# imedslab/OAProgressionMMF

Measured on AMD Instinct MI355X. Metric: knees/sec full XR+MRI+clin fusion train step, higher is better.
Workload: dtype f32; 1 GPU; syn3: XR1MR3C1CnnTrf train step (fwd+FocalLoss+bwd+Adam), per-GPU batch 8, global batch 8, BASELINE config 4 on BASELINE's synthetic tensors: XR 1x310x310 + 3 x MRI 1x160x384x384 (slice-major) + 9 clinical; random-init weights; parallelism=dp1, activation_recompute=012,012,01

## Files before the change

oaprogressionmmf_amd/csrc/koaf_conv.hip:

```cpp
#include <string.h>
#include "koaf_common.h"
#include <stdlib.h>

namespace {

inline void zero_gemm(KoafGemm* g) { *g = KoafGemm{}; g->alpha = 1.f; g->nb0 = g->nb1 = 1; g->splitk = 1; }

inline int conv_out(int H, int K, int s, int p) { return (H + 2 * p - K) / s + 1; }

inline int64_t rup32(int64_t v) { return (v + 31) / 32 * 32; }

inline void set_fimg(KoafGemm* g, const KoafWImg* w, int R, int64_t K) {
    g->fmt = 1;
    g->A.fscale = KOAF_ACT_SCALE;
    g->B.amax = w->amax;
    if (!w->f) return;
    g->B.kind = 2; g->B.gather = 0;
    g->B.planes = w->f; g->B.ld = rup32(K); g->B.plane_stride = (int64_t)R * g->B.ld;
}

inline void set_aplanes(KoafOperand* a, const uint16_t* planes, int64_t plane_elems) {
    a->kind = 2; a->planes = planes; a->plane_stride = plane_elems; a->zeros = planes + 2 * plane_elems;
    a->ptr = nullptr; a->ptr2 = nullptr; a->tf = 0; a->sc = a->sh = a->sc2 = nullptr;
}
// ... 253 lines not shown
        g.A.ld = Cin;
    } else {
        g.A.gather = 1;
        g.A.H = H; g.A.W = W; g.A.C = Cin; g.A.CS = Cin;
        g.A.PH = OH; g.A.PW = OW;
        g.A.KH = KH; g.A.KW = KW; g.A.stride = stride; g.A.pad = pad; g.A.pad_w = pad;
    }
    if (in_sc) { g.A.tf = 1; g.A.sc = in_sc; g.A.sh = in_sh; }
    if (tail) { g.A.tf = 3; g.A.ptr2 = tail->idt; g.A.side = tail->y_out; g.A.sc2 = tail->idt_sc; g.A.sh2 = tail->idt_sc ? tail->idt_sh : nullptr; }
    g.B.ptr = w;
    g.B.kind = 0;
    g.B.ld = (int64_t)KH * KW * Cin;
    g.M = (int)M; g.N = Cout; g.K = KH * KW * Cin;
    if (wimg && wimg->amax) set_fimg(&g, wimg, Cout, g.K);
    if (x_planes) {
        KOAF_REQUIRE(g.A.gather == 1 && g.B.kind == 2, "koaf_conv2d_fwd: x_planes serve the gathered kernels and need wimg->f");
        set_aplanes(&g.A, x_planes, (int64_t)N * H * W * Cin);
    }
    g.C = y; g.ldc = Cout;
    g.stats = stats;
    g.stats_shift = stats ? stats_shift : nullptr;
    g.act16 = act16 ? 1 : 0;
    if (emit) {
        KOAF_REQUIRE(emit->planes && emit->sc && emit->sh && (Cout % 8) == 0, "koaf_conv2d_fwd: emit needs planes / sc / sh and Cout %% 8 == 0");
        g.out_planes = emit->planes; g.out_sc = emit->sc; g.out_sh = emit->sh; g.out_ps = M * Cout;
    }
    if (stats_rows) *stats_rows = koaf_gemm_part_rows(&g);
    return koaf_gemm(&g, stream);
}

extern "C" int32_t koaf_conv2d_stats_rows(int64_t M, int32_t Cout) { return (int32_t)cdiv64(M, 64); }

static void set_apply(KoafOperand* a, const KoafBnApply* ap, int C) {
    a->ptr = ap->dz; a->ptr2 = ap->c; a->tf = 2;
    a->sc = ap->coef; a->sc2 = ap->coef + 2 * (int64_t)C; a->sh = ap->coef + 3 * (int64_t)C;
    a->amax = ap->amax;
}

static void set_bnb(KoafGemm* g, const KoafBnb* b, float* part) {
    if (!b) return;
    g->bnb_amax = b->dz_amax;
    g->bnb_mode = b->mode;
    g->bnb_c = b->c; g->bnb_y = b->y; g->bnb_sc = b->sc; g->bnb_sh = b->sh;
    g->bnb_mean = b->mean; g->bnb_invstd = b->invstd;
    g->bnb2_c = b->c2; g->bnb2_mean = b->mean2; g->bnb2_invstd = b->invstd2;
    g->bnb_part = part;
}

extern "C" int32_t koaf_conv2d_dgrad_bnb_rows(int32_t N, int32_t H, int32_t W, int32_t Cin, int32_t stride) {
    if (stride == 2) {
        int64_t r = 0;
        for (int py = 0; py < 2; ++py)
            for (int px = 0; px < 2; ++px) r += cdiv64((int64_t)N * ((H - py + 1) / 2) * ((W - px + 1) / 2), 64);
        return (int32_t)r;
    }
    return (int32_t)cdiv64((int64_t)N * H * W, 64);
}

extern "C" int koaf_conv2d_dgrad_bnb(const float* dy, const float* w, float* dx, int32_t N, int32_t H, int32_t W,
                                     int32_t Cin, int32_t Cout, int32_t KH, int32_t KW, int32_t stride, int32_t pad,
                                     const float* residual, const KoafBnb* bnb, float* part, int32_t* part_rows,
                                     const KoafWImg* wimg, const float* dy_amax, const KoafBnApply* dy_apply,
                                     const uint16_t* dy_planes, int32_t act16, void* stream) {
    KOAF_REQUIRE(!dy_planes || (wimg && wimg->amax && wimg->d && (dy_amax || dy_apply) && KH * KW > 1),
                 "koaf_conv2d_dgrad: dy_planes need the weight's D plane image, dy_amax and a gathered (KH*KW > 1) kernel");
    KOAF_REQUIRE((dy || dy_apply || dy_planes) && w && dx && N > 0 && Cout % 32 == 0 && Cin % 4 == 0, "koaf_conv2d_dgrad: bad args");
    KOAF_REQUIRE(!dy_apply || (dy_apply->dz && dy_apply->c && dy_apply->coef && dy_apply->amax && wimg && wimg->amax && wimg->d),
                 "koaf_conv2d_dgrad: dy_apply needs dz / c / coef / amax and the weight's D plane image");
    if (dy_apply) { dy = dy_apply->dz; dy_amax = dy_apply->amax; }
    if (bnb && bnb->dz_amax && hipMemsetAsync(bnb->dz_amax, 0, sizeof(float), (hipStream_t)stream) != hipSuccess) {
        koaf_set_error("koaf_conv2d_dgrad_bnb: memset failed");
        return KOAF_ELAUNCH;
    }
    const bool f16 = wimg && wimg->amax && dy_amax;
    const bool ps = f16 && wimg->d != nullptr;
    const uint16_t* w_dimg = ps ? wimg->d : nullptr;
    const int64_t dld = (int64_t)KH * KW * Cout, dps = (int64_t)Cin * dld;
    KOAF_REQUIRE(!bnb || (part && part_rows), "koaf_conv2d_dgrad_bnb: part / part_rows required");
    const int nsum = (bnb && bnb->c2) ? 3 : 2;
    int rows_done = 0;
    const int OH = conv_out(H, KH, stride, pad), OW = conv_out(W, KW, stride, pad);
    const int64_t M = (int64_t)N * H * W;
    KOAF_REQUIRE(M < (1ll << 31), "koaf_conv2d_dgrad: too many pixels");
    KoafGemm g;
    if (stride == 2) {
        for (int py = 0; py < 2; ++py)
            for (int px = 0; px < 2; ++px) {
                const int Hc = (H - py + 1) / 2, Wc = (W - px + 1) / 2;
                if (Hc <= 0 || Wc <= 0) continue;
                const int khs = (py + pad) & 1, kws = (px + pad) & 1;
                const int nkh = khs < KH ? (KH - khs + 1) / 2 : 0, nkw = kws < KW ? (KW - kws + 1) / 2 : 0;
                const int offy = (py + pad - khs) / 2, offx = (px + pad - kws) / 2;
                zero_gemm(&g);
                g.prec = 1;
                if (f16) { g.fmt = 1; g.A.amax = dy_amax; g.B.amax = wimg->amax; }
                g.A.ptr = dy; g.A.kind = 0; g.A.gather = 2;
                if (dy_apply) set_apply(&g.A, dy_apply, Cout);
                g.A.H = OH; g.A.W = OW; g.A.C = Cout; g.A.CS = Cout;
                g.A.PH = Hc; g.A.PW = Wc;
                g.A.KH = nkh > 0 ? nkh : 1; g.A.KW = nkw > 0 ? nkw : 1; g.A.stride = 1; g.A.pad = offy; g.A.pad_w = offx;
                g.B.ptr = w + ((int64_t)khs * KW + kws) * Cin; g.B.kind = 1; g.B.gather = 3;
                g.B.C = Cout; g.B.ld = (int64_t)KH * KW * Cin;
                g.B.KW = g.A.KW; g.B.tap_stride = 2ll * Cin; g.B.tap_stride_h = 2ll * KW * Cin;
                if (ps) {
                    g.B.kind = 2; g.B.gather = 0;
                    g.B.planes = w_dimg + ((int64_t)khs * KW + kws) * Cout; g.B.ld = dld; g.B.plane_stride = dps;
                    g.B.tap_stride = 2ll * Cout; g.B.tap_stride_h = 2ll * KW * Cout;
                }
                if (dy_planes && nkh > 0 && nkw > 0) set_aplanes(&g.A, dy_planes, (int64_t)N * OH * OW * Cout);
                g.M = N * Hc * Wc; g.N = Cin; g.K = nkh * nkw * Cout;
                g.C = dx; g.ldc = Cin;
                g.residual = residual; g.ldr = Cin;
                g.cmap = 1; g.cm_PH = Hc; g.cm_PW = Wc; g.cm_H = H; g.cm_W = W; g.cm_py = py; g.cm_px = px;
                if (bnb) {
                    set_bnb(&g, bnb, part + (int64_t)rows_done * nsum * Cin);
                    rows_done += koaf_gemm_part_rows(&g);
                }
                g.act16 = act16 ? 2 : 0;
                int rc = koaf_gemm(&g, stream);
                if (rc != KOAF_OK) return rc;
            }
        if (part_rows) *part_rows = rows_done;
        return KOAF_OK;
    }
    zero_gemm(&g);
    g.prec = 1;
    if (f16) { g.fmt = 1; g.A.amax = dy_amax; g.B.amax = wimg->amax; }
    g.A.ptr = dy;
    g.A.kind = 0;
    if (dy_apply) set_apply(&g.A, dy_apply, Cout);
    g.B.ptr = w;
    g.B.kind = 1;
    if (KH == 1 && KW == 1 && stride == 1 && pad == 0) {
        g.A.gather = 0;
        g.A.ld = Cout;
        g.B.gather = 0;
        g.B.ld = Cin;
    } else {
        g.A.gather = 2;
        g.A.H = OH; g.A.W = OW; g.A.C = Cout; g.A.CS = Cout;
        g.A.PH = H; g.A.PW = W;
        g.A.KH = KH; g.A.KW = KW; g.A.stride = stride; g.A.pad = pad; g.A.pad_w = pad;
        g.B.gather = 3;
        g.B.C = Cout;
        g.B.ld = (int64_t)KH * KW * Cin;
        g.B.KW = KW;
        g.B.tap_stride = Cin;
        g.B.tap_stride_h = (int64_t)KW * Cin;
    }
    if (ps) {
        g.B.kind = 2; g.B.gather = 0; g.B.C = 0; g.B.tap_stride = g.B.tap_stride_h = 0;
        g.B.planes = w_dimg; g.B.ld = dld; g.B.plane_stride = dps;
    }
    if (dy_planes) set_aplanes(&g.A, dy_planes, (int64_t)N * OH * OW * Cout);
    g.M = (int)M; g.N = Cin; g.K = KH * KW * Cout;
    g.C = dx; g.ldc = Cin;
    g.residual = residual; g.ldr = Cin;
    if (bnb) {
        set_bnb(&g, bnb, part);
        *part_rows = koaf_gemm_part_rows(&g);
    }
    g.act16 = act16 ? 2 : 0;
    return koaf_gemm(&g, stream);
}

extern "C" int koaf_conv2d_dgrad(const float* dy, const float* w, float* dx, int32_t N, int32_t H, int32_t W,
                                 int32_t Cin, int32_t Cout, int32_t KH, int32_t KW, int32_t stride, int32_t pad,
                                 const float* residual, const KoafWImg* wimg, const float* dy_amax,
                                 const KoafBnApply* dy_apply, const uint16_t* dy_planes, int32_t act16, void* stream) {
    return koaf_conv2d_dgrad_bnb(dy, w, dx, N, H, W, Cin, Cout, KH, KW, stride, pad, residual, nullptr, nullptr,
                                 nullptr, wimg, dy_amax, dy_apply, dy_planes, act16, stream);
}

bool koaf_wgrad3_ring_ok(int N, int H, int W, int Cin, int Cout);
int64_t koaf_wgrad3_ring_ws(int N, int H, int W, int Cin, int Cout);
// ... 453 lines not shown
```

oaprogressionmmf_amd/models/_encoder.py:

```python
import os
from collections import namedtuple

import torch
from torch import nn

from .. import ops
from ..arena import deliver_grad, grad_target, packed_weight, weight_planes
from ._core_fes import BasicBlock, Bottleneck

USE_SIDE_STREAM = os.environ.get("KOAF_SIDE_STREAM", "1") != "0"


class _Rec:
    __slots__ = ("kind", "blk", "yin", "c1", "s1", "c2", "s2", "c3", "s3", "cd", "sd", "y", "dims", "wexp", "tail")

    def __init__(self):
        for k in self.__slots__:
            setattr(self, k, None)


def _stat_shift(bn, train):
    return bn.running_mean if (train and bn is not None and bn.running_mean is not None) else None


# ... 32 lines not shown
                                      tail_idsaved=tail.idsaved, emit=emit)
    elif g == 1:
        y, part = ops.conv2d_fwd(x, w, N, H, W, cin, cout, k, k, s, p, sc, sh, stats=train, shift=shift,
                                 wimg=weight_planes(conv.weight), keep_planes=keep_planes, emit=emit)
    else:
        if k != 3 or p != 1 or cin != cout:
            raise NotImplementedError("grouped convolution other than the ResNeXt 3x3 is not built")
        wexp = ops.gconv_expand_w(w, cin, g)
        y, part = ops.gconv3x3_fwd(x, wexp, N, H, W, cin, s, sc, sh, stats=train, shift=shift)
    return y, part, ops.conv_out(H, k, s, p), ops.conv_out(W, k, s, p), wexp, yin


def _bn_fin(bn, part, count):
    train = bn.training or bn.running_mean is None
    return ops.bn_finalize(part if train else None, bn.num_features, count, bn.weight.detach(), bn.bias.detach(),
                           bn.running_mean, bn.running_var, bn.num_batches_tracked if train else None,
                           -1.0 if bn.momentum is None else bn.momentum, bn.eps, train, shift=_stat_shift(bn, train))


_LANES = {}


def lane_streams(device, lane):
    key = (device.index, lane)
    if key not in _LANES:
        _LANES[key] = (torch.cuda.Stream(device=device, priority=0), torch.cuda.Stream(device=device, priority=0))
    return _LANES[key]


_JOIN = {"queued": False, "streams": []}
CALLER_STREAM = None


def _final_join():
    for st, caller in _JOIN["streams"]:
        (caller if caller is not None else torch.cuda.current_stream()).wait_stream(st)
    _JOIN["streams"] = []
    _JOIN["queued"] = False


def _register_join(stream, caller=None):
    _JOIN["streams"].append((stream, caller))
    if not _JOIN["queued"]:
        _JOIN["queued"] = True
        from torch.autograd import Variable
        Variable._execution_engine.queue_callback(_final_join)


class _SideStream:
    _streams = {}

    def __init__(self, device, stream=None, hold=False):
        if stream is None:
            key = (device.type, device.index)
            if key not in _SideStream._streams:
                _SideStream._streams[key] = torch.cuda.Stream(device=device, priority=0)
            stream = _SideStream._streams[key]
        self.stream = stream
        self.pending = []
        self.hold = hold
        self.held = []

    def run(self, inputs, fn, param, buf, acc):
        main = torch.cuda.current_stream()
        self.stream.wait_stream(main)
        with torch.cuda.stream(self.stream):
            fn()
        if self.hold:
            self.held.append(inputs)
        else:
            for t in inputs:
                if t is not None:
                    t.record_stream(self.stream)
        self.pending.append((param, buf, acc))

    def join(self):
        torch.cuda.current_stream().wait_stream(self.stream)
        for param, buf, acc in self.pending:
            deliver_grad(param, buf, acc)
        self.pending = []
        self.held = []


def _conv_bwd(conv, dc, x, N, H, W, in_saved, wexp, residual=None, need_dx=True, side=None, bnb=None):
    w = packed_weight(conv.weight)
    cin, cout = conv.in_channels, conv.out_channels
    k, s, p, g = conv.kernel_size[0], conv.stride[0], conv.padding[0], conv.groups
    wimg = weight_planes(conv.weight) if g == 1 else None
    if isinstance(dc, ops.BnApply) and (g != 1 or (need_dx and wimg is None)):
        dc = dc.materialize(want_amax=True)
    amax = getattr(dc, "_koaf_amax", None)
    sc, sh = (in_saved[2], in_saved[3]) if in_saved is not None else (None, None)
    need_dw = conv.weight.requires_grad
    gw, acc = grad_target(conv.weight) if need_dw else (None, False)
    if not need_dw:
        side = None

    def wgrad():
        if g == 1:
            ops.conv2d_wgrad(dc, x, gw, N, H, W, cin, cout, k, k, s, p, sc, sh, dy_amax=amax)
        else:
            dwexp = ops.gconv3x3_wgrad(dc, x, N, H, W, cin, s, sc, sh)
            ops.gconv_compress_dw(dwexp, gw, cin, g)
    if side is None and need_dw:
        wgrad()
        deliver_grad(conv.weight, gw, acc)
    dx = part = dzmax = None
    if need_dx:
        if g != 1:
            assert residual is None and bnb is None
            dx = ops.gconv3x3_dgrad(dc, wexp, N, H, W, cin, s)
        else:
            res = ops.conv2d_dgrad(dc, w, N, H, W, cin, cout, k, k, s, p, residual=residual, bnb=bnb, wimg=wimg, dy_amax=amax)
            if bnb is None:
                dx = res
            elif bnb.get("dz_amax"):
                dx, part, dzmax = res
            else:
                dx, part = res
    if side is not None:
        held = dc.tensors() if isinstance(dc, ops.BnApply) else (dc, amax)
        side.run(held + (x, in_saved), wgrad, conv.weight, gw, acc)
    return dx, part, dzmax


def _bn_train(bn):
    return bn.training or bn.running_mean is None


def _bn_grad_targets(bn):
    return (grad_target(bn.weight) if bn.weight.requires_grad else (None, False),
            grad_target(bn.bias) if bn.bias.requires_grad else (None, False))


def _bn_deliver(bn, gg, ag, gb, ab):
    if gg is not None:
        deliver_grad(bn.weight, gg, ag)
    if gb is not None:
        deliver_grad(bn.bias, gb, ab)


def _bn_bwd(bn, g, c, saved, rows, mask_mode=None, ymask=None, dz_out=None, dc_out=None, pool=None, part=None, dzmax=None):
    C = bn.num_features
    (gg, ag), (gb, ab) = _bn_grad_targets(bn)
    train = _bn_train(bn)
    if part is not None:
        fused = ops.CONV_F16 and dzmax is not None
        dc = ops.bn_bwd_from_part(*part, g, c, saved, rows, C, rows, gg, gb, dc_out=None if fused else dc_out,
                                  fused=fused, dzmax=dzmax, train=train)
    else:
        dc = ops.bn_bwd(g, c, saved, rows, C, rows, gg, gb, mask_mode, ymask=ymask, dz_out=dz_out,
                        fused=pool is not None or ops.CONV_F16, pool=pool, train=train)
    _bn_deliver(bn, gg, ag, gb, ab)
    return dc


_Pend = namedtuple("_Pend", "part nsum dzmax")


def _bnb(mode, c, saved, y=None, cd=None, sd=None):
    d = dict(mode=mode, c=c, saved=saved, y=y, dz_amax=ops.CONV_F16)
    if cd is not None:
        d["c2"], d["saved2"] = cd, sd
    return d


def _tail_bnb(prev):
    if prev is None:
        return None
    c_last, s_last = (prev.c3, prev.s3) if prev.kind == "bottleneck" else (prev.c2, prev.s2)
    return _bnb(1, c_last, s_last, y=prev.y, cd=prev.cd, sd=prev.sd)


def _conv_bn_bwd(conv, slot, bn, c, saved, N, H, W, side, wexp=None, epilogue=True):
    dz, part, dzmax = _conv_bwd(conv, slot.pop(), c, N, H, W, saved, wexp, side=side, bnb=_bnb(2, c, saved) if epilogue else None)
    return _bn_bwd(bn, dz, c, saved, N * H * W, 2, dc_out=dz, part=None if part is None else (part, 2, 1), dzmax=dzmax)


def _block_fwd(blk, y, N, Hc, Wc, train, given, tail=None, defer=False, skip_tail=False):
    r = _Rec()
    r.blk, r.yin = blk, y
    want = train and given is None

    def fin(bn, part, count, idx):
        return given[idx] if given is not None else _bn_fin(bn, part, count)
    if isinstance(blk, Bottleneck):
        r.kind = "bottleneck"
        s1_pre, emit = None, None
        if not want and _takes_planes(blk.conv2) and blk.conv1.groups == 1 and weight_planes(blk.conv1.weight) is not None:
            s1_pre = fin(blk.bn1, None, N * Hc * Wc, 0)
            emit = (s1_pre[2], s1_pre[3])
        if tail is not None:
            r.c1, part, _, _, _, y = _conv_fwd(tail.c, blk.conv1, N, Hc, Wc, tail.saved, want, blk.bn1, tail=tail, emit=emit)
            r.yin = y
        else:
            r.c1, part, _, _, _, _ = _conv_fwd(y, blk.conv1, N, Hc, Wc, None, want, blk.bn1, emit=emit)
        r.s1 = s1_pre if s1_pre is not None else fin(blk.bn1, part, N * Hc * Wc, 0)
        r.c2, part, OH, OW, r.wexp, _ = _conv_fwd(r.c1, blk.conv2, N, Hc, Wc, r.s1, want, blk.bn2, keep_planes=given is not None)
        r.s2 = fin(blk.bn2, part, N * OH * OW, 1)
        r.c3, part, _, _, _, _ = _conv_fwd(r.c2, blk.conv3, N, OH, OW, r.s2, want, blk.bn3)
        r.s3 = fin(blk.bn3, part, N * OH * OW, 2)
        last_c, last_s, cout = r.c3, r.s3, blk.conv3.out_channels
    elif isinstance(blk, BasicBlock):
        r.kind = "basic"
        r.c1, part, OH, OW, _, _ = _conv_fwd(y, blk.conv1, N, Hc, Wc, None, want, blk.bn1)
        r.s1 = fin(blk.bn1, part, N * OH * OW, 0)
        r.c2, part, _, _, _, _ = _conv_fwd(r.c1, blk.conv2, N, OH, OW, r.s1, want, blk.bn2)
        r.s2 = fin(blk.bn2, part, N * OH * OW, 1)
        last_c, last_s, cout = r.c2, r.s2, blk.conv2.out_channels
    else:
        raise TypeError(f"unsupported block {type(blk)}")
    rows_o = N * OH * OW
    idt, idsaved = y, None
    if blk.downsample is not None:
        r.cd, part, _, _, _, _ = _conv_fwd(y, blk.downsample[0], N, Hc, Wc, None, want, blk.downsample[1])
        r.sd = fin(blk.downsample[1], part, rows_o, 3)
        idt, idsaved = r.cd, r.sd
    if skip_tail:
        pass
    elif defer:
        r.tail = _Tail(last_c, last_s, idt, torch.empty_like(last_c), idsaved)
    else:
        r.y = ops.bn_add_relu(last_c, last_s, rows_o, cout, idt=idt, idsaved=idsaved)
    r.dims = (N, Hc, Wc, OH, OW)
    return r


def _blocks_fwd(blocks, y, N, Hc, Wc, train, givens=None, tail=None, defer_last=False, slim=False, last_y=None):
    recs, yin0 = [], None
    for i, blk in enumerate(blocks):
        nxt = blocks[i + 1] if i + 1 < len(blocks) else None
        defer = (nxt is not None and _can_take_tail(nxt)) or (nxt is None and defer_last)
        have = nxt is None and last_y is not None
        r = _block_fwd(blk, y, N, Hc, Wc, train, givens[i] if givens is not None else None, tail=tail, defer=defer, skip_tail=have)
        if have:
            r.y = last_y
        if i == 0:
            yin0 = r.yin
        if recs:
            if tail is not None:
# ... 54 lines not shown
        for si, stage in enumerate(st["stages"]):
            rec_stage = si in rset
            defer_last = si + 1 < nst and _can_take_tail(st["stages"][si + 1][0])
            recs, y_out, Ho, Wo, yin0 = _blocks_fwd(stage, y, N, Hc, Wc, train, tail=tail, defer_last=defer_last, slim=rec_stage or not keep)
            if tail is not None:
                y = yin0
                if prev_recs:
                    prev_recs[-1].y = y
            sv = dict(yin=y if rec_stage else None, H=Hc, W=Wc, stats=[], recs=[], recompute=rec_stage)
            if rec_stage:
                sv["stats"] = [(r.s1, r.s2, r.s3, r.sd) for r in recs]
            elif keep:
                sv["recs"] = recs
            tail = recs[-1].tail
            prev_recs = sv["recs"]
            if rec_stage or not keep:
                for r in recs:
                    r.c1 = r.c2 = r.c3 = r.cd = r.yin = r.y = None
            del recs
            y, Hc, Wc = y_out, Ho, Wo
            stages_saved.append(sv)
        C = y.shape[-1]
        if trunk.keep_features:
            if CALLER_STREAM is not None:
                y.record_stream(CALLER_STREAM)
            trunk.features = (y, N, Hc, Wc, C)
        if st["gap"]:
            out = ops.gap_fwd(y, N, Hc * Wc, C).view(N, C, 1, 1)
        else:
            out = y.permute(0, 3, 1, 2)
            if out.dtype != torch.float32:
                out = out.float()
        if keep:
            if 0 in rset:
                c0 = None
            ctx.state = dict(x=x, c0=c0, s0=s0, am=am, stages=stages_saved, any_recompute=bool(rset), caller=CALLER_STREAM,
                             block_level=block_level, adt=adt,
                             dims=(N, H, W, H1, W1), last=(Hc, Wc, C), st=st, lane=lane, train=train, xshape=xshape)
        return out

    @staticmethod
    def backward(ctx, gout):
        S = ctx.state
        ctx.state = None
        lane = S["lane"]
        need_dx = ctx.needs_input_grad[0]
        if lane is None:
            return EncoderFn._backward_body(S, gout, None, need_dx)
        main_s, side_s = lane_streams(gout.device, lane)
        cur = torch.cuda.current_stream()
        if cur != main_s:
            main_s.wait_stream(cur)
            gout.record_stream(main_s)
        with torch.cuda.stream(main_s):
            out = EncoderFn._backward_body(S, gout, side_s, need_dx)
        if out[0] is not None and cur != main_s:
            cur.wait_stream(main_s)
            out[0].record_stream(cur)
        _register_join(main_s, S.get("caller"))
        return out

    @staticmethod
    def _blocks_bwd(recs, dy, side):
        pend = None
        while recs:
            r = recs.pop()
            prev = recs[-1] if recs else None
            blk = r.blk
            N, Hi, Wi, OH, OW = r.dims
            rows_o = N * OH * OW
            bott = r.kind == "bottleneck"
            tail_bn = blk.bn3 if bott else blk.bn2
            tail_c, tail_s = (r.c3, r.s3) if bott else (r.c2, r.s2)
            if pend is None:
                slot = [_bn_bwd(tail_bn, dy, tail_c, tail_s, rows_o, 1, ymask=r.y, dz_out=dy)]
            else:
                slot = [_bn_bwd(tail_bn, dy, tail_c, tail_s, rows_o, part=(pend.part, pend.nsum, 1), dzmax=pend.dzmax)]
            dz = dy
            if bott:
                slot = [_conv_bn_bwd(blk.conv3, slot, blk.bn2, r.c2, r.s2, N, OH, OW, side)]
                slot = [_conv_bn_bwd(blk.conv2, slot, blk.bn1, r.c1, r.s1, N, Hi, Wi, side, wexp=r.wexp, epilogue=blk.conv2.groups == 1)]
            else:
                slot = [_conv_bn_bwd(blk.conv2, slot, blk.bn1, r.c1, r.s1, N, OH, OW, side)]
            if blk.downsample is not None:
                if pend is None:
                    dcd = _bn_bwd(blk.downsample[1], dz, r.cd, r.sd, rows_o, 0)
                else:
                    dcd = _bn_bwd(blk.downsample[1], dz, r.cd, r.sd, rows_o, dc_out=dz, part=(pend.part, pend.nsum, 2), dzmax=pend.dzmax)
                resid = _conv_bwd(blk.downsample[0], dcd, r.yin, N, Hi, Wi, None, None, side=side)[0]
            else:
                resid = dz
            bnb = _tail_bnb(prev)
            dy, part, dzmax = _conv_bwd(blk.conv1, slot.pop(), r.yin, N, Hi, Wi, None, None, residual=resid, side=side, bnb=bnb)
            pend = _Pend(part, 3 if "c2" in bnb else 2, dzmax) if bnb is not None else None
            del dz, resid, r
            if side is not None and side.hold:
                side.join()
        return dy

    @staticmethod
    def _backward_body(S, gout, side_stream, need_dx=False):
        st = S["st"]
        N, H, W, H1, W1 = S["dims"]
        Hc, Wc, C = S["last"]
        if st["gap"]:
            dy = ops.gap_bwd(gout.reshape(N, C).contiguous(), N, Hc * Wc, C).view(N, Hc, Wc, C)
        else:
            dy = gout.permute(0, 2, 3, 1).contiguous()
            if dy.data_ptr() == gout.data_ptr():
                dy = dy.clone()
        side = _SideStream(gout.device, side_stream, hold=S["any_recompute"]) if USE_SIDE_STREAM else None
        stages = st["stages"]
        run = []
        next_in = None
        for si in range(len(stages) - 1, -1, -1):
            sv = S["stages"][si]
            if not sv["recompute"]:
                run = sv["recs"] + run
                sv["recs"] = None
                if si > 0 and not S["stages"][si - 1]["recompute"]:
                    continue
                first_in = run[0].yin
                dy = EncoderFn._blocks_bwd(run, dy, side)
                run = []
                next_in = first_in
                continue
            y, Hc2, Wc2 = sv["yin"], sv["H"], sv["W"]
            sv["yin"] = None
            stage_in, last_y = y, next_in
            next_in = None
            if S["block_level"] and len(stages[si]) > 1:
                ins = [(y, Hc2, Wc2)]
                for blk, given in zip(stages[si][:-1], sv["stats"][:-1]):
                    r = _block_fwd(blk, y, N, Hc2, Wc2, S["train"], given)
                    y, Hc2, Wc2 = r.y, r.dims[3], r.dims[4]
                    ins.append((y, Hc2, Wc2))
                    del r
                for bi in range(len(stages[si]) - 1, -1, -1):
                    yb, hb, wb = ins.pop()
                    r = _block_fwd(stages[si][bi], yb, N, hb, wb, S["train"], sv["stats"][bi])
                    dy = EncoderFn._blocks_bwd([r], dy, side)
                    del r, yb
                del y, last_y
                next_in = stage_in
                continue
            recs, y, Hc2, Wc2, _ = _blocks_fwd(stages[si], y, N, Hc2, Wc2, S["train"], givens=sv["stats"], last_y=last_y)
            del last_y
            dy = EncoderFn._blocks_bwd(recs, dy, side)
            del recs, y
            next_in = stage_in
        next_in = None
        conv1, bn1 = st["conv1"], st["bn1"]
        need_dw = conv1.weight.requires_grad
        if not (need_dx or need_dw or bn1.weight.requires_grad or bn1.bias.requires_grad):
            if side is not None:
                side.join()
            return None, None, None, None, None
        c0 = S["c0"]
        w1t = ops.stem_fold_w(packed_weight(conv1.weight)) if (c0 is None or need_dx) else None
        if c0 is None:
            c0 = ops.stem_fwd(S["x"], w1t, N, H, W, dtype=S["adt"])
        dc0 = _bn_bwd(bn1, None, c0, S["s0"], N * H1 * W1, 2, pool=(dy, S["am"], N, H1, W1))
        if need_dw:
            gw, acc = grad_target(conv1.weight)
            ops.stem_wgrad(dc0, S["x"], gw, N, H, W)
            deliver_grad(conv1.weight, gw, acc)
        dx = ops.stem_dgrad(dc0, w1t, N, H, W).view(S["xshape"]) if need_dx else None
        if side is not None:
            side.join()
        return dx, None, None, None, None


class KoafTrunk(nn.Sequential):
    act_dtype = torch.float32
    keep_features = False
    features = None

    def _koaf_layout(self):
# ... 30 lines not shown
```

oaprogressionmmf_amd/ops.py:

```python
import ctypes

import torch

from ._lib import KoafBnApply, KoafBnb, KoafEmit, KoafGemm, KoafError, KoafLaunchRec, KoafTail, KoafWImg, KoafWPlane, check, defines, lib

_i32 = ctypes.c_int32

import os
CONV_F16 = os.environ.get("KOAF_CONV_FMT", "f16") != "bf16"
APLANES_MASK = int(os.environ.get("KOAF_APLANES", "7"))
APLANES = APLANES_MASK != 0
ACT_SCALE = defines()["KOAF_ACT_SCALE"]
KEEP_XPLANES_ELEMS = int(os.environ.get("KOAF_KEEP_XPLANES_ELEMS", "0"))

PROFILE = None


def _prof_begin():
    if PROFILE is None:
        return None
    e = torch.cuda.Event(enable_timing=True)
    e.record()
    return e

# ... 111 lines not shown


def conv_out(h, k, s, p):
    return (h + 2 * p - k) // s + 1


def act_planes(x, npix, C, tf=0, sc=None, sh=None, x2=None, sc2=None, amax=None, fscale=0.0):
    L = lib()
    out = torch.empty(L.koaf_act_planes_elems(npix, C), device=x.device, dtype=torch.int16)
    check(L.koaf_act_planes(_ptr(x), _ptr(x2), npix, C, tf, _ptr(sc), _ptr(sh), _ptr(sc2), _ptr(amax), float(fscale),
                            out.data_ptr(), _a16(x2 if tf == 2 else x), _stream()), "act_planes")
    return out


def set_conv3x3_halo(mode):
    return lib().koaf_set_conv3x3_halo(int(mode))


def set_stream(on):
    return bool(lib().koaf_set_stream(1 if on else 0))


def launch_log(on):
    return bool(lib().koaf_launch_log(1 if on else 0))


def launch_log_read():
    L = lib()
    n = min(L.koaf_launch_log_read(None, 0), 4096)
    buf = (KoafLaunchRec * max(n, 1))()
    L.koaf_launch_log_read(buf, n)
    return [{f: (getattr(r, f).decode() if f == "variant" else getattr(r, f)) for f, _ in KoafLaunchRec._fields_} for r in buf[:n]]


def use_aplanes(wimg, KH, KW, C):
    return APLANES and wimg is not None and KH * KW > 1 and C % 32 == 0


def conv2d_fwd(x, w, N, H, W, Cin, Cout, KH, KW, stride, pad, in_sc=None, in_sh=None, stats=False, shift=None, wimg=None,
               aplanes=None, tail_idt=None, tail_out=None, tail_idsaved=None, keep_planes=False, emit=None):
    L = lib()
    OH, OW = conv_out(H, KH, stride, pad), conv_out(W, KW, stride, pad)
    if tail_idt is not None and tail_out is None:
        tail_out = torch.empty_like(x)
    y = _empty((N, OH, OW, Cout), x, dtype=x.dtype)
    part, rows = None, _i32(0)
    if stats:
        nrows = L.koaf_conv2d_stats_rows(N * OH * OW, Cout)
        part = _empty((nrows, 2, Cout), x)
    e0 = _prof_begin()
    if aplanes is None:
        aplanes = (APLANES_MASK & 1) and use_aplanes(wimg, KH, KW, Cin) and wimg[0] is not None and stride == 1
    xpl = None
    tail = None
    if tail_idt is not None:
        tail = ctypes.byref(KoafTail(idt=_ptr(tail_idt), y_out=_ptr(tail_out),
                                     idt_sc=_ptr(tail_idsaved[2]) if tail_idsaved is not None else None,
                                     idt_sh=_ptr(tail_idsaved[3]) if tail_idsaved is not None else None))
        aplanes = False
    if torch.is_tensor(aplanes):
        xpl = aplanes
    elif aplanes:
        ep = getattr(x, "_koaf_eplanes", None)
        if ep is not None:
            del x._koaf_eplanes
        if (ep is not None and in_sc is not None and ep[1].data_ptr() == in_sc.data_ptr() and ep[2].data_ptr() == in_sh.data_ptr()
                and ep[0].numel() == L.koaf_act_planes_elems(N * H * W, Cin)):
            xpl = ep[0]
        else:
            xpl = act_planes(x, N * H * W, Cin, 1 if in_sc is not None else 0, in_sc, in_sh, fscale=ACT_SCALE)
    epl, em = None, None
    if emit is not None:
        epl = torch.empty(L.koaf_act_planes_elems(N * OH * OW, Cout), device=x.device, dtype=torch.int16)
        em = ctypes.byref(KoafEmit(planes=epl.data_ptr(), sc=_ptr(emit[0]), sh=_ptr(emit[1])))
    check(L.koaf_conv2d_fwd(_ptr(x), _ptr(w), _ptr(y), N, H, W, Cin, Cout, KH, KW, stride, pad, _ptr(in_sc),
                            _ptr(in_sh), _ptr(part), ctypes.addressof(rows), _ptr(shift) if stats else None,
                            _img(wimg), xpl.data_ptr() if xpl is not None else None, tail, em, _a16(x), _stream()), "conv2d_fwd")
    if epl is not None:
        y._koaf_eplanes = (epl, emit[0], emit[1])
    if xpl is not None and not torch.is_tensor(aplanes) and (keep_planes or xpl.numel() <= KEEP_XPLANES_ELEMS):
        y._koaf_xplanes = xpl
    _prof_end(e0, "gemm", 2.0 * N * OH * OW * Cout * KH * KW * Cin,
              f"conv_fwd k{KH}s{stride} {Cin}->{Cout} px{N*OH*OW}" + (" +tail" if tail is not None else ""),
              N * H * W * Cin * (3 if tail is not None else 1) + Cout * KH * KW * Cin + N * OH * OW * Cout * (2 if epl is not None else 1),
              mpp=3 if wimg is not None else 6)
    if stats:
        part = part[:rows.value]
    if tail is not None:
        return y, part, tail_out
    return y, part


def conv2d_dgrad(dy, w, N, H, W, Cin, Cout, KH, KW, stride, pad, residual=None, bnb=None, wimg=None, dy_amax=None,
                 aplanes=None):
    L = lib()
    dyp, amp, app, like = _dy_args(dy, dy_amax)
    a16 = _a16(dy.c) if isinstance(dy, BnApply) else (_a16(bnb["c"]) if bnb is not None else 0)
    dx = _empty((N, H, W, Cin), like)
    if aplanes is None:
        aplanes = ((APLANES_MASK & 2) and use_aplanes(wimg, KH, KW, Cout) and wimg[1] is not None and stride in (1, 2) and
                   (app is not None or dy_amax is not None))
    e0 = _prof_begin()
    dypl = None
    if aplanes:
        dypl = _dy_planes(dy, dy_amax, N * conv_out(H, KH, stride, pad) * conv_out(W, KW, stride, pad), Cout)
    dypp = dypl.data_ptr() if dypl is not None else None
    fl = 2.0 * N * conv_out(H, KH, stride, pad) * conv_out(W, KW, stride, pad) * Cout * KH * KW * Cin
    tag = f"conv_dgrad k{KH}s{stride} {Cin}->{Cout} px{N*H*W}"
    el = N * conv_out(H, KH, stride, pad) * conv_out(W, KW, stride, pad) * Cout + Cout * KH * KW * Cin + N * H * W * Cin
    el += N * H * W * Cin if residual is not None else 0
    mpp = 3 if (wimg is not None and (dy_amax is not None or app is not None)) else 6
    if app is not None:
        el += N * conv_out(H, KH, stride, pad) * conv_out(W, KW, stride, pad) * Cout
        tag += " apply"
    if bnb is None:
        check(L.koaf_conv2d_dgrad(dyp, _ptr(w), _ptr(dx), N, H, W, Cin, Cout, KH, KW, stride, pad,
                                  _ptr(residual), _img(wimg), amp, app, dypp, a16, _stream()), "conv2d_dgrad")
        _prof_end(e0, "gemm", fl, tag, el, mpp=mpp)
        return dx
    sv, sv2 = bnb["saved"], bnb.get("saved2")
    dzmax = _empty((1,), like) if bnb.get("dz_amax") else None
    kb = KoafBnb(mode=bnb["mode"], dz_amax=_ptr(dzmax), c=_ptr(bnb["c"]), y=_ptr(bnb.get("y")), sc=_ptr(sv[2]), sh=_ptr(sv[3]),
                 mean=_ptr(sv[0]), invstd=_ptr(sv[1]), c2=_ptr(bnb.get("c2")),
                 mean2=_ptr(sv2[0]) if sv2 is not None else None, invstd2=_ptr(sv2[1]) if sv2 is not None else None)
    nsum = 3 if bnb.get("c2") is not None else 2
    part = _empty((L.koaf_conv2d_dgrad_bnb_rows(N, H, W, Cin, stride), nsum, Cin), like)
    rows = _i32(0)
    check(L.koaf_conv2d_dgrad_bnb(dyp, _ptr(w), _ptr(dx), N, H, W, Cin, Cout, KH, KW, stride, pad,
                                  _ptr(residual), ctypes.byref(kb), _ptr(part), ctypes.addressof(rows), _img(wimg),
                                  amp, app, dypp, a16, _stream()), "conv2d_dgrad_bnb")
    el += N * H * W * Cin * (1 + (bnb.get("y") is not None) + (bnb.get("c2") is not None))
    _prof_end(e0, "gemm", fl, tag + " +bnb", el, mpp=mpp)
    if dzmax is not None:
        return dx, part[:rows.value], dzmax
    return dx, part[:rows.value]


def _dy_planes(dy, dy_amax, npo, Cout):
    if isinstance(dy, BnApply):
        if dy._koaf_planes is None:
            dy._koaf_planes = act_planes(dy.dz, npo, Cout, 2, dy.coef[0], dy.coef[3], x2=dy.c, sc2=dy.coef[2], amax=dy.amax)
        return dy._koaf_planes
    return act_planes(dy, npo, Cout, 0, amax=dy_amax)


def _slab_ws(slabs, ws, like, what):
    if slabs is None:
        return _empty((ws,), like) if ws > 0 else None
    if not slabs.is_cuda or slabs.dtype != torch.float32 or not slabs.is_contiguous() or slabs.numel() < ws:
        raise KoafError(f"{what}: the slab workspace is a contiguous fp32 device tensor of at least {ws} elements")
    return slabs


def conv2d_wgrad(dy, x, dw, N, H, W, Cin, Cout, KH, KW, stride, pad, in_sc=None, in_sh=None, dy_amax=None, aplanes=None,
                 slabs=None):
    L = lib()
    dyp, amp, app, like = _dy_args(dy, dy_amax)
    slabs = _slab_ws(slabs, L.koaf_conv2d_wgrad_ws(N, H, W, Cin, Cout, KH, KW, stride, pad), like, "conv2d_wgrad")
    if aplanes is None:
        aplanes = ((APLANES_MASK & 4) and KH * KW > 1 and stride == 1 and Cin % 8 == 0 and Cout % 8 == 0 and
                   (app is not None or dy_amax is not None))
    e0 = _prof_begin()
    dypl = xpl = None
    if aplanes:
        npo = N * conv_out(H, KH, stride, pad) * conv_out(W, KW, stride, pad)
        dypl = _dy_planes(dy, dy_amax, npo, Cout)
        xpl = getattr(dy.c, "_koaf_xplanes", None) if app is not None else None
        if xpl is None or xpl.numel() != L.koaf_act_planes_elems(N * H * W, Cin):
            xpl = act_planes(x, N * H * W, Cin, 1 if in_sc is not None else 0, in_sc, in_sh, fscale=ACT_SCALE)
    check(L.koaf_conv2d_wgrad(dyp, _ptr(x), _ptr(dw), N, H, W, Cin, Cout, KH, KW, stride, pad, _ptr(in_sc),
                              _ptr(in_sh), _ptr(slabs), amp, app, dypl.data_ptr() if dypl is not None else None,
                              xpl.data_ptr() if xpl is not None else None, _a16(x), _stream()), "conv2d_wgrad")
    npx = N * conv_out(H, KH, stride, pad) * conv_out(W, KW, stride, pad)
    _prof_end(e0, "gemm", 2.0 * npx * Cout * KH * KW * Cin,
              f"conv_wgrad k{KH}s{stride} {Cin}->{Cout} px{N*H*W}" + (" apply" if app is not None else ""),
              npx * Cout * (2 if app is not None else 1) + N * H * W * Cin + Cout * KH * KW * Cin,
              mpp=3 if (dy_amax is not None or app is not None) else 6)
    return dw


def gconv_expand_w(w, C, groups):
    wexp = _empty((C // 64, 64, 9, 64), w)
    amax = torch.zeros(1, device=w.device, dtype=torch.float32) if CONV_F16 else None
    check(lib().koaf_gconv_expand_w(_ptr(w), _ptr(wexp), C, groups, _ptr(amax), _stream()), "gconv_expand_w")
    if amax is not None:
        wexp._koaf_amax = amax
    return wexp


def gconv_compress_dw(dwexp, dw, C, groups):
    check(lib().koaf_gconv_compress_dw(_ptr(dwexp), _ptr(dw), C, groups, _stream()), "gconv_compress_dw")
    return dw

# ... 732 lines not shown
```

Baseline: 4.029 knees/s.

## Accumulate strided 1x1 shortcut dgrad in place into conv1 dx

For downsample blocks with a 1x1 stride-2 shortcut on large tensors, conv1's dgrad now runs first. The shortcut dgrad then accumulates into that dx buffer in place, touching only the stride-2 phase that has taps and skipping the zero phases. This avoids materialising a full-resolution shortcut gradient and re-reading it as a residual. In exchange, the fused bnb epilogue for conv1 is not used on this path, and correctness relies on residual == dx aliasing in the GEMM.

```diff
diff --git a/oaprogressionmmf_amd/csrc/koaf_conv.hip b/oaprogressionmmf_amd/csrc/koaf_conv.hip
--- a/oaprogressionmmf_amd/csrc/koaf_conv.hip
+++ b/oaprogressionmmf_amd/csrc/koaf_conv.hip
@@ -359,6 +359,8 @@
     const int OH = conv_out(H, KH, stride, pad), OW = conv_out(W, KW, stride, pad);
     const int64_t M = (int64_t)N * H * W;
     KOAF_REQUIRE(M < (1ll << 31), "koaf_conv2d_dgrad: too many pixels");
+    const bool inplace = residual != nullptr && residual == dx;
+    KOAF_REQUIRE(!inplace || (stride == 2 && !bnb), "koaf_conv2d_dgrad: residual == dx (accumulate in place) serves stride 2 without bnb");
     KoafGemm g;
     if (stride == 2) {
         for (int py = 0; py < 2; ++py)
@@ -368,6 +370,24 @@
                 const int khs = (py + pad) & 1, kws = (px + pad) & 1;
                 const int nkh = khs < KH ? (KH - khs + 1) / 2 : 0, nkw = kws < KW ? (KW - kws + 1) / 2 : 0;
                 const int offy = (py + pad - khs) / 2, offx = (px + pad - kws) / 2;
+                if (inplace && (nkh == 0 || nkw == 0)) continue;
+                if (inplace && KH == 1 && KW == 1 && pad == 0 && !dy_planes) {
+                    zero_gemm(&g);
+                    g.prec = 1;
+                    if (f16) { g.fmt = 1; g.A.amax = dy_amax; g.B.amax = wimg->amax; }
+                    g.A.ptr = dy; g.A.kind = 0; g.A.gather = 0; g.A.ld = Cout;
+                    if (dy_apply) set_apply(&g.A, dy_apply, Cout);
+                    g.B.ptr = w; g.B.kind = 1; g.B.gather = 0; g.B.ld = Cin;
+                    if (ps) { g.B.kind = 2; g.B.planes = w_dimg; g.B.ld = dld; g.B.plane_stride = dps; }
+                    g.M = N * Hc * Wc; g.N = Cin; g.K = Cout;
+                    g.C = dx; g.ldc = Cin;
+                    g.residual = residual; g.ldr = Cin;
+                    g.cmap = 1; g.cm_PH = Hc; g.cm_PW = Wc; g.cm_H = H; g.cm_W = W; g.cm_py = py; g.cm_px = px;
+                    g.act16 = act16 ? 2 : 0;
+                    int rc = koaf_gemm(&g, stream);
+                    if (rc != KOAF_OK) return rc;
+                    continue;
+                }
                 zero_gemm(&g);
                 g.prec = 1;
                 if (f16) { g.fmt = 1; g.A.amax = dy_amax; g.B.amax = wimg->amax; }
diff --git a/oaprogressionmmf_amd/models/_encoder.py b/oaprogressionmmf_amd/models/_encoder.py
--- a/oaprogressionmmf_amd/models/_encoder.py
+++ b/oaprogressionmmf_amd/models/_encoder.py
@@ -138,7 +138,7 @@
         self.held = []
 
 
-def _conv_bwd(conv, dc, x, N, H, W, in_saved, wexp, residual=None, need_dx=True, side=None, bnb=None):
+def _conv_bwd(conv, dc, x, N, H, W, in_saved, wexp, residual=None, need_dx=True, side=None, bnb=None, out=None):
     w = packed_weight(conv.weight)
     cin, cout = conv.in_channels, conv.out_channels
     k, s, p, g = conv.kernel_size[0], conv.stride[0], conv.padding[0], conv.groups
@@ -164,10 +164,10 @@
     dx = part = dzmax = None
     if need_dx:
         if g != 1:
-            assert residual is None and bnb is None
+            assert residual is None and bnb is None and out is None
             dx = ops.gconv3x3_dgrad(dc, wexp, N, H, W, cin, s)
         else:
-            res = ops.conv2d_dgrad(dc, w, N, H, W, cin, cout, k, k, s, p, residual=residual, bnb=bnb, wimg=wimg, dy_amax=amax)
+            res = ops.conv2d_dgrad(dc, w, N, H, W, cin, cout, k, k, s, p, residual=residual, bnb=bnb, wimg=wimg, dy_amax=amax, out=out)
             if bnb is None:
                 dx = res
             elif bnb.get("dz_amax"):
@@ -212,6 +212,18 @@
 
 
 _Pend = namedtuple("_Pend", "part nsum dzmax")
+
+
+SHORTCUT_INPLACE = True
+SHORTCUT_INPLACE_MIN_BYTES = 64 << 20
+
+
+def _shortcut_inplace(blk, dcd, bnb, nbytes):
+    if not SHORTCUT_INPLACE or bnb is not None or blk.downsample is None or nbytes < SHORTCUT_INPLACE_MIN_BYTES:
+        return False
+    ds = blk.downsample[0]
+    return (ds.kernel_size == (1, 1) and ds.stride == (2, 2) and ds.padding == (0, 0) and ds.groups == 1 and
+            (isinstance(dcd, ops.BnApply) or getattr(dcd, "_koaf_amax", None) is not None))
 
 
 def _bnb(mode, c, saved, y=None, cd=None, sd=None):
@@ -432,18 +444,22 @@
                 slot = [_conv_bn_bwd(blk.conv2, slot, blk.bn1, r.c1, r.s1, N, Hi, Wi, side, wexp=r.wexp, epilogue=blk.conv2.groups == 1)]
             else:
                 slot = [_conv_bn_bwd(blk.conv2, slot, blk.bn1, r.c1, r.s1, N, OH, OW, side)]
+            bnb = _tail_bnb(prev)
+            dcd = None
             if blk.downsample is not None:
                 if pend is None:
                     dcd = _bn_bwd(blk.downsample[1], dz, r.cd, r.sd, rows_o, 0)
                 else:
                     dcd = _bn_bwd(blk.downsample[1], dz, r.cd, r.sd, rows_o, dc_out=dz, part=(pend.part, pend.nsum, 2), dzmax=pend.dzmax)
-                resid = _conv_bwd(blk.downsample[0], dcd, r.yin, N, Hi, Wi, None, None, side=side)[0]
+            if _shortcut_inplace(blk, dcd, bnb, 4 * r.yin.numel()):
+                dy, part, dzmax = _conv_bwd(blk.conv1, slot.pop(), r.yin, N, Hi, Wi, None, None, side=side)
+                _conv_bwd(blk.downsample[0], dcd, r.yin, N, Hi, Wi, None, None, side=side, out=dy)
+                resid = None
             else:
-                resid = dz
-            bnb = _tail_bnb(prev)
-            dy, part, dzmax = _conv_bwd(blk.conv1, slot.pop(), r.yin, N, Hi, Wi, None, None, residual=resid, side=side, bnb=bnb)
+                resid = _conv_bwd(blk.downsample[0], dcd, r.yin, N, Hi, Wi, None, None, side=side)[0] if dcd is not None else dz
+                dy, part, dzmax = _conv_bwd(blk.conv1, slot.pop(), r.yin, N, Hi, Wi, None, None, residual=resid, side=side, bnb=bnb)
             pend = _Pend(part, 3 if "c2" in bnb else 2, dzmax) if bnb is not None else None
-            del dz, resid, r
+            del dz, resid, dcd, r
             if side is not None and side.hold:
                 side.join()
         return dy
diff --git a/oaprogressionmmf_amd/ops.py b/oaprogressionmmf_amd/ops.py
--- a/oaprogressionmmf_amd/ops.py
+++ b/oaprogressionmmf_amd/ops.py
@@ -217,7 +217,7 @@
         y._koaf_xplanes = xpl
     _prof_end(e0, "gemm", 2.0 * N * OH * OW * Cout * KH * KW * Cin,
               f"conv_fwd k{KH}s{stride} {Cin}->{Cout} px{N*OH*OW}" + (" +tail" if tail is not None else ""),
-              N * H * W * Cin * (3 if tail is not None else 1) + Cout * KH * KW * Cin + N * OH * OW * Cout * (2 if epl is not None else 1),
+              (N * OH * OW if (KH == 1 and KW == 1 and pad == 0) else N * H * W) * Cin * (3 if tail is not None else 1) + Cout * KH * KW * Cin + N * OH * OW * Cout * (2 if epl is not None else 1),
               mpp=3 if wimg is not None else 6)
     if stats:
         part = part[:rows.value]
@@ -227,11 +227,18 @@
 
 
 def conv2d_dgrad(dy, w, N, H, W, Cin, Cout, KH, KW, stride, pad, residual=None, bnb=None, wimg=None, dy_amax=None,
-                 aplanes=None):
+                 aplanes=None, out=None):
     L = lib()
     dyp, amp, app, like = _dy_args(dy, dy_amax)
     a16 = _a16(dy.c) if isinstance(dy, BnApply) else (_a16(bnb["c"]) if bnb is not None else 0)
-    dx = _empty((N, H, W, Cin), like)
+    if out is not None:
+        if residual is not None or bnb is not None or stride != 2:
+            raise KoafError("conv2d_dgrad: out= (accumulate in place) serves stride 2 without residual / bnb")
+        if not out.is_cuda or out.dtype != torch.float32 or not out.is_contiguous() or out.numel() != N * H * W * Cin:
+            raise KoafError("conv2d_dgrad: out= must be a contiguous fp32 [N,H,W,Cin] device tensor")
+        dx = residual = out
+    else:
+        dx = _empty((N, H, W, Cin), like)
     if aplanes is None:
         aplanes = ((APLANES_MASK & 2) and use_aplanes(wimg, KH, KW, Cout) and wimg[1] is not None and stride in (1, 2) and
                    (app is not None or dy_amax is not None))
@@ -244,6 +251,10 @@
     tag = f"conv_dgrad k{KH}s{stride} {Cin}->{Cout} px{N*H*W}"
     el = N * conv_out(H, KH, stride, pad) * conv_out(W, KW, stride, pad) * Cout + Cout * KH * KW * Cin + N * H * W * Cin
     el += N * H * W * Cin if residual is not None else 0
+    if out is not None:
+        tag += " inplace"
+        if KH == 1 and KW == 1 and pad == 0:
+            el += 2 * Cin * (N * conv_out(H, 1, 2, 0) * conv_out(W, 1, 2, 0) - N * H * W)
     mpp = 3 if (wimg is not None and (dy_amax is not None or app is not None)) else 6
     if app is not None:
         el += N * conv_out(H, KH, stride, pad) * conv_out(W, KW, stride, pad) * Cout
```

New measurement: 4.065 knees/s, median of 6. No clear change (+0.9%).
